# HKUST-Aerial-Robotics/ESVO

Hardware: AMD Instinct MI355X
Metric: mapped events/sec (stereo TS raster + block matching + LM depth refinement + fusion), events resident in HBM before the timed region; exactly K ticks between two synchronisations, i.e. including the fill and the drain of the two-deep tick pipeline (`sustained`: the same workload over 1600 ticks) (higher is better)
Workload: dtype f64

## Files before the change

esvo_amd/csrc/kernels_lm.hip:

```cpp
#define DEV_HOOKS_LM_TU
#include "common.hpp"
#include "dev_hooks.hpp"
#include "fdiv.hpp"
#include "lm_common.hpp"


namespace esvo {

#define LM_ROWS 7
#define LM_COLS 15

template <int CTRL>
__device__ inline double dpp_f64(double v) {
  const int lo = __double2loint(v), hi = __double2hiint(v);
  const int lo2 = __builtin_amdgcn_update_dpp(0, lo, CTRL, 0xf, 0xf, true);
  const int hi2 = __builtin_amdgcn_update_dpp(0, hi, CTRL, 0xf, 0xf, true);
  return __hiloint2double(hi2, lo2);
}
template <int CTRL>
__device__ inline int dpp_i32(int v) { return __builtin_amdgcn_update_dpp(0, v, CTRL, 0xf, 0xf, true); }
#define DPP_XOR1 0xB1
#define DPP_XOR2 0x4E
#define DPP_HALF_MIRROR 0x141
#define DPP_MIRROR 0x140
#define DPP_SHL1 0x101

__device__ inline double grp_sum(double v) {
  v = v + dpp_f64<DPP_XOR1>(v);
  v = v + dpp_f64<DPP_XOR2>(v);
  v = v + dpp_f64<DPP_HALF_MIRROR>(v);
  v = v + dpp_f64<DPP_MIRROR>(v);
  return v;
}
__device__ inline int grp_sum_int(int v) {
  v += dpp_i32<DPP_XOR1>(v);
  v += dpp_i32<DPP_XOR2>(v);
  v += dpp_i32<DPP_HALF_MIRROR>(v);
  v += dpp_i32<DPP_MIRROR>(v);
  return v;
}
__device__ inline double grp_min(double v) {
  v = fmin(v, dpp_f64<DPP_XOR1>(v));
  v = fmin(v, dpp_f64<DPP_XOR2>(v));
  v = fmin(v, dpp_f64<DPP_HALF_MIRROR>(v));
  v = fmin(v, dpp_f64<DPP_MIRROR>(v));
  return v;
}
template <bool WIDE>
struct Lay {
  static constexpr int RL = WIDE ? 2 : LM_ROWS;
};
__device__ inline double hop_f64(double v, int k) {
  const u32 lo = (u32)__double2loint(v), hi = (u32)__double2hiint(v);
  u32 l2, h2;
  if (k == 2) {
    l2 = __builtin_amdgcn_permlane32_swap(lo, lo, false, false)[0];
    h2 = __builtin_amdgcn_permlane32_swap(hi, hi, false, false)[0];
  } else if (k == 1) {
    l2 = __builtin_amdgcn_permlane16_swap(lo, lo, false, false)[0];
    h2 = __builtin_amdgcn_permlane16_swap(hi, hi, false, false)[0];
  } else {
    l2 = __builtin_amdgcn_permlane16_swap(lo, lo, false, false)[1];
    h2 = __builtin_amdgcn_permlane16_swap(hi, hi, false, false)[1];
  }
  return __hiloint2double((int)h2, (int)l2);
}
#define LM_WIDE_LAST_ROW_LANE 32
__device__ inline double bcast_f64(double v, int lane) {
  return __hiloint2double(__builtin_amdgcn_readlane(__double2hiint(v), lane), __builtin_amdgcn_readlane(__double2loint(v), lane));
}
template <bool WIDE>
__device__ inline double patch_sum(const double* t, int rg) {
  if constexpr (!WIDE) {
    double a = t[0];
#pragma unroll
    for (int y = 1; y < LM_ROWS; ++y) a = a + t[y];
    return grp_sum(a);
  } else {
    double a = t[0] + t[1];
    a = (hop_f64(a, 1) + t[0]) + t[1];
    a = (hop_f64(a, 2) + t[0]) + t[1];
    a = hop_f64(a, 3) + t[0];
    (void)rg;
    return bcast_f64(grp_sum(a), LM_WIDE_LAST_ROW_LANE);
  }
}
template <bool WIDE>
__device__ inline int match_sum_int(int v) {
  v = grp_sum_int(v);
  if constexpr (WIDE)
    v = (__builtin_amdgcn_readlane(v, 0) + __builtin_amdgcn_readlane(v, 16)) + (__builtin_amdgcn_readlane(v, 32) + __builtin_amdgcn_readlane(v, 48));
  return v;
}
template <bool WIDE>
__device__ inline double match_min(double v) {
  v = grp_min(v);
  if constexpr (WIDE) v = fmin(fmin(bcast_f64(v, 0), bcast_f64(v, 16)), fmin(bcast_f64(v, 32), bcast_f64(v, 48)));
  return v;
}
template <bool WIDE>
__device__ inline double patch_dot(const double* a, const double* b, int rg) {
  double t[Lay<WIDE>::RL];
#pragma unroll
  for (int y = 0; y < Lay<WIDE>::RL; ++y) t[y] = a[y] * b[y];
  return patch_sum<WIDE>(t, rg);
}

__device__ inline double in_vgpr(double x) {
  asm volatile("" : "+v"(x));
  return x;
}

struct LmProblem {
  double T[12];
  double cx, cy;
  double ray[3];
  __amdgpu_buffer_rsrc_t tsL;
  __amdgpu_buffer_rsrc_t tsR;
  const double* cam;
  int c;
  int rg;
  int vy0, vy1;
  DEV_LM_PROBLEM_FIELDS
};

struct PatchGeom { int ulx, uly; double q1, q2, q3, q4; bool ok; };
__device__ inline PatchGeom interp_geom(const DevParams& p, double lx, double ly) {
  PatchGeom g;
  const int hx = (LM_COLS - 1) / 2, hy = (LM_ROWS - 1) / 2;
  const double fx = floor(lx), fy = floor(ly);
  const int l1 = (int)fx, l0 = (int)fy;
  g.ulx = l1 - hx;
  g.uly = l0 - hy;
  const int drx = l1 + hx, dry = l0 + hy;
  g.ok = (int)(g.ulx >= 0) & (int)(g.uly >= 0) & (int)(drx < p.W) & (int)(dry < p.H) & (int)(g.uly + LM_ROWS < p.H) & (int)(g.ulx + LM_COLS < p.W);
  g.q1 = (fx + 1.0) - lx;
  g.q2 = lx - fx;
  g.q3 = (fy + 1.0) - ly;
  g.q4 = ly - fy;
  return g;
}
template <bool WIDE>
struct LmCache {
  float l[Lay<WIDE>::RL + 1], r[Lay<WIDE>::RL + 1];
  int vl, vr;
  __device__ inline void clear() {
#pragma unroll
    for (int y = 0; y <= Lay<WIDE>::RL; ++y) l[y] = r[y] = 0.f;
    vl = vr = 0x7fffffff;
  }
};
__device__ inline float dpp_shl1_f32(float v) { return __int_as_float(dpp_i32<DPP_SHL1>(__float_as_int(v))); }
template <bool WIDE>
__device__ inline void interp_column(__amdgpu_buffer_rsrc_t img, int W, const PatchGeom& g, int c, int rg, double* tau, float* cs,
                                     int& cvoff) {
  constexpr int RL = Lay<WIDE>::RL;
  const int voff = (g.uly + (WIDE ? 2 * rg : 0)) * W + g.ulx + c;
  if (__ballot(voff != cvoff) != 0ull) {
#pragma unroll
    for (int y = 0; y <= RL; ++y) cs[y] = (float)(int)__builtin_amdgcn_raw_buffer_load_b8(img, voff, y * W, 0);
    cvoff = voff;
  }
  double R[RL + 1];
#pragma unroll
  for (int y = 0; y <= RL; ++y) {
    const float s0 = cs[y];
    const float s1 = dpp_shl1_f32(s0);
    R[y] = g.q1 * (double)s0 + g.q2 * (double)s1;
  }
#pragma unroll
  for (int y = 0; y < RL; ++y) tau[y] = g.q3 * R[y] + g.q4 * R[y + 1];
}

template <bool WIDE, bool L2, bool COUNT = false, bool BAND = false>
__device__ bool lm_eval(const DevParams& p, const LmProblem& pr, LmCache<WIDE>& cc, double x, double* fv, int* n_iter = nullptr,
                        bool* viol = nullptr) {
  int iters = 0;
  constexpr int RL = Lay<WIDE>::RL;
  bool el[RL];
#pragma unroll
  for (int y = 0; y < RL; ++y) el[y] = pr.c < LM_COLS && (!WIDE || 2 * pr.rg + y < LM_ROWS);
  const double nu = in_vgpr(p.td_nu);
  DEV_LM_EVAL(pr);
  if constexpr (WIDE) asm volatile("" ::: "memory");
  double prv[3], pl[3];
  {
    const double z = 1.0 / x;
#pragma unroll
    for (int r = 0; r < 3; ++r) prv[r] = z * pr.ray[r] - pr.cam[24 + r];
  }
#pragma unroll
  for (int r = 0; r < 3; ++r)
    pl[r] = ((pr.T[r * 4 + 0] * prv[0] + pr.T[r * 4 + 1] * prv[1]) + pr.T[r * 4 + 2] * prv[2]) + pr.T[r * 4 + 3];
  double x1u, x1v, x2u, x2v;
  {
    double hL[3], hR[3];
#pragma unroll
    for (int r = 0; r < 3; ++r) {
      const double* PL = pr.cam + r * 4;
      const double* PR = pr.cam + 12 + r * 4;
      hL[r] = ((PL[0] * pl[0] + PL[1] * pl[1]) + PL[2] * pl[2]) + PL[3];
      hR[r] = ((PR[0] * pl[0] + PR[1] * pl[1]) + PR[2] * pl[2]) + PR[3];
    }
    if (__double_as_longlong(hL[2]) == __double_as_longlong(hR[2]) &&
        (unsigned)(((__double2hiint(hL[2]) >> 20) & 0x7ff) - 923) <= 200u) {
      Recip rz;
      rz.b = hL[2];
      rz.y = recip_refined(hL[2]);
      x1u = div_fast(hL[0], rz);
      x1v = div_fast(hL[1], rz);
      x2u = div_fast(hR[0], rz);
      x2v = div_fast(hR[1], rz);
    } else {
      x1u = hL[0] / hL[2];
      x1v = hL[1] / hL[2];
      x2u = hR[0] / hR[2];
      x2v = hR[1] / hR[2];
    }
  }
  const int hx = (LM_COLS - 1) / 2, hy = (LM_ROWS - 1) / 2;
  const double wlo = (double)hx, whi = (double)(p.W - hx), vlo = (double)hy, vhi = (double)(p.H - hy);
  const bool inside = (int)(x1u >= wlo) & (int)(x1u <= whi) & (int)(x1v >= vlo) & (int)(x1v <= vhi) &
                      (int)(x2u >= wlo) & (int)(x2u <= whi) & (int)(x2v >= vlo) & (int)(x2v <= vhi);
  const PatchGeom g1 = interp_geom(p, x1u, x1v), g2 = interp_geom(p, x2u, x2v);
  const bool okw = inside & g1.ok & g2.ok;
  if constexpr (BAND) {
    const bool bad = (int)okw & ((int)(g1.uly < pr.vy0) | (int)(g1.uly + LM_ROWS >= pr.vy1) | (int)(g2.uly < pr.vy0) | (int)(g2.uly + LM_ROWS >= pr.vy1));
    *viol = *viol | bad;
  }
  double tau1[RL], tau2[RL], r[RL], r2[RL];
  interp_column<WIDE>(pr.tsL, p.W, g1, pr.c, pr.rg, tau1, cc.l, cc.vl);
  interp_column<WIDE>(pr.tsR, p.W, g2, pr.c, pr.rg, tau2, cc.r, cc.vr);
  if (!okw) {
    double f = 255;
    if constexpr (!L2) {
      const double q = f / p.td_scale;
      const double weight = (nu + 1) / (nu + q * q);
      f = sqrt(weight) * f;
    }
#pragma unroll
    for (int y = 0; y < RL; ++y) fv[y] = el[y] ? f : 0.0;
    if constexpr (COUNT) *n_iter = 0;
    return false;
  }
  if constexpr (L2) {
#pragma unroll
    for (int y = 0; y < RL; ++y) fv[y] = el[y] ? (tau1[y] - tau2[y]) : 0.0;
    return false;
  }
  int knz = 0;
  double minabs = 1e300, r2max = 0;
  double r2n[RL];
#pragma unroll
  for (int y = 0; y < RL; ++y) {
    r[y] = el[y] ? (tau1[y] - tau2[y]) : 0.0;
    r2[y] = r[y] * r[y];
    r2n[y] = r2[y] * (nu + 1);
    r2max = fmax(r2max, r2[y]);
    if (r[y] != 0) { knz++; minabs = fmin(minabs, fabs(r[y])); }
  }
  const int knz_lane = knz;
  knz = match_sum_int<WIDE>(knz);
  DEV_LM_FIRST_EVAL_KNZ(pr, knz);
  minabs = match_min<WIDE>(minabs);
  const double scale2_0 = in_vgpr(p.td_scale2);
  double s2;
  const int e_r2max = (__double2hiint(r2max) >> 20) & 0x7ff;
  const bool r2_tight = knz_lane == 0 || (minabs * minabs >= 0x1p-100 && r2max < 0x1p98);
  const bool nu_mid = nu >= 0x1p-100 && nu < 0x1p100;
  bool lane_ok = r2_tight && nu_mid;
  if (!lane_ok) {
    bool r2_ok = true;
#pragma unroll
    for (int y = 0; y < RL; ++y) r2_ok = r2_ok && fdiv_ok(r2[y]);
    lane_ok = r2_ok && fdiv_ok(nu) && nu > 0 && fdiv_ok(r2max * (nu + 1));
  }
  const int N = LM_ROWS * LM_COLS;
  const bool tight = match_sum_int<WIDE>((r2_tight && nu_mid) ? 0 : 1) == 0;
  if ((double)knz * (nu + 1) / (double)N <= 0.94 && minabs >= 1e-6) {
    s2 = scale2_0;
    DEV_LM_SHORTCUT(pr);
  } else {
    double s1 = scale2_0;
    const Recip rN = make_recip((double)N);
    bool done = false;
    if (tight) {
      while ((unsigned)(((__double2hiint(s1) >> 20) & 0xfff) - 923) <= 200u) {
        if constexpr (COUNT) ++iters;
        DEV_LM_SCALE_ITER(pr);
        Recip rs1;
        rs1.b = s1;
        rs1.y = recip_refined(s1);
        double t[RL];
#pragma unroll
        for (int y = 0; y < RL; ++y) {
          Recip rd;
          rd.b = nu + div_fast(r2[y], rs1);
          rd.y = recip_refined(rd.b);
          t[y] = div_fast(r2n[y], rd);
        }
        const double sum = patch_sum<WIDE>(t, pr.rg);
        if (sum == 0) { s2 = scale2_0; done = true; break; }
        s2 = div_fast(sum, rN);
        const double rel = div_fast(fabs(s2 - s1), rs1);
        if (!(rel > 0.05)) { done = true; break; }
        s1 = s2;
      }
    }
    while (!done) {
      if constexpr (COUNT) ++iters;
      DEV_LM_SCALE_ITER(pr);
      double t[RL];
      const Recip rs1 = make_recip(s1);
      const int e_s1 = (__double2hiint(s1) >> 20) & 0x7ff;
      if (lane_ok && rs1.fast && s1 > 0 && e_r2max - e_s1 < 300) {
#pragma unroll
        for (int y = 0; y < RL; ++y)
          t[y] = div_fast(r2n[y], make_recip(nu + div_fast(r2[y], rs1)));
      } else {
#pragma unroll
        for (int y = 0; y < RL; ++y) t[y] = (r[y] != 0) ? r2[y] * (nu + 1) / (nu + r2[y] / s1) : 0.0;
      }
      const double sum = patch_sum<WIDE>(t, pr.rg);
      if (sum == 0) { s2 = scale2_0; break; }
      s2 = div_by(sum, rN);
      const double rel = div_by(fabs(s2 - s1), rs1);
      if (!(rel > 0.05)) break;
      s1 = s2;
    }
  }
  if (tight && (unsigned)(((__double2hiint(s2) >> 20) & 0xfff) - 923) <= 200u) {
    Recip rs2;
    rs2.b = s2;
    rs2.y = recip_refined(s2);
    const double nu1 = nu + 1;
#pragma unroll
    for (int y = 0; y < RL; ++y) {
      Recip rd;
      rd.b = nu + div_fast(r2[y], rs2);
      rd.y = recip_refined(rd.b);
      fv[y] = sqrt_moderate(div_fast(nu1, rd)) * r[y];
    }
    if constexpr (COUNT) *n_iter = iters;
    return true;
  }
  const Recip rs2 = make_recip(s2);
  const bool fast2 = lane_ok && rs2.fast && s2 > 0 && e_r2max - ((__double2hiint(s2) >> 20) & 0x7ff) < 300;
#pragma unroll
  for (int y = 0; y < RL; ++y) {
    fv[y] = fast2 ? sqrt_moderate(div_fast(nu + 1, make_recip(nu + div_fast(r2[y], rs2)))) * r[y]
                  : sqrt((nu + 1) / (nu + r2[y] / s2)) * r[y];
  }
  if constexpr (COUNT) *n_iter = iters;
  return false;
}

#ifndef LM_WAVES
#define LM_WAVES 2
#endif
#ifndef LM_BLOCK
#define LM_BLOCK 64
#endif
#ifndef LM_WIDE_WAVES
#define LM_WIDE_WAVES 3
#endif
#ifndef LM_WIDE_MAX
#define LM_WIDE_MAX 40000u
#endif
struct LmSplit {
  double* fvec0;
  double* fnorm0;
  u32* meta;
  u32* order;
  u32* hist;
};
#define LM_SPLIT_BINS 64
#define LM_SPLIT_STRIPES 32
__device__ inline u32 lm_split_stripe(u32 slot) { return (slot >> 2) & (LM_SPLIT_STRIPES - 1); }

template <bool WIDE, bool L2 = false, int STAGE = 0, bool PAIR = false, bool BAND = false>
__global__ void __launch_bounds__(PAIR ? 128 : LM_BLOCK, WIDE ? LM_WIDE_WAVES : LM_WAVES) lm_refine_kernel(LmArgs a, DevParams p, u32* n_solved, LmSplit sp) {
  static_assert(!PAIR || (WIDE && !L2 && STAGE == 0), "the pair layout is a variant of the wide one");
  static_assert(!BAND || (STAGE == 0 && !PAIR), "routed band launches are single launches of the narrow or the wide layout");
  constexpr int RL = Lay<WIDE>::RL;
  __shared__ double lds_pair[PAIR ? 2 : 1][2][RL][64];
  __shared__ int lds_pair_tight[PAIR ? 2 : 1][2];
  const int wv = PAIR ? (int)(threadIdx.x >> 6) : 0;
  const int ln = threadIdx.x & 63;
  __shared__ double lds_cam[28];
  if (threadIdx.x < 27) {
    const int i = threadIdx.x;
    lds_cam[i] = i < 12 ? p.camL.P[i] : (i < 24 ? p.camR.P[i - 12] : p.camL.Kinv_t[i - 24]);
  }
  __syncthreads();
  const u32 pos = WIDE ? blockIdx.x : (blockIdx.x * LM_BLOCK + threadIdx.x) >> 4;
  const int c = threadIdx.x & 15;
  const int drow = (threadIdx.x >> 4) & 3;
  const int rg = WIDE ? (drow ^ (drow >> 1)) : 0;
  const bool lead = WIDE ? threadIdx.x == 0 : c == 0;
  u32 M = *a.n_matches;
  if (M > a.max_matches) M = a.max_matches;
  bool active = pos < M;
  u32 s = pos;
  if constexpr (STAGE == 2) {
    if (blockIdx.x < 2 * LM_SPLIT_STRIPES * LM_SPLIT_BINS / LM_BLOCK) sp.hist[blockIdx.x * LM_BLOCK + threadIdx.x] = 0u;
    s = active ? sp.order[pos] : 0xffffffffu;
  }
  if (STAGE != 2 && !active && lead && s < a.max_matches) a.out_flags[s] = 0u;
  if (__ballot(active) == 0) return;
  const bool probe = STAGE != 1 && a.clk != nullptr && threadIdx.x == 0 && blockIdx.x % CLK_STRIDE == 0u;
  if (probe) {
    u64* sc = a.clk + CLK_SCRATCH + 2 * (size_t)(blockIdx.x / CLK_STRIDE);
    sc[0] = __builtin_readcyclecounter();
    sc[1] = __builtin_amdgcn_s_memrealtime();
  }
  u32 j = 0;
  esvo_match_t m;
  m.x_left[0] = m.x_left[1] = -1e9; m.inv_depth = 1.0; m.pose_idx = 0; m.cost = 0; m.disp = 0; m.event_idx = 0;
  if (active) {
    j = a.dense ? s : stride_item(s, M, (u32)p.num_threads);
    u32 jm = j;
    if constexpr (WIDE) { if (a.match_index) jm = a.match_index[j]; }
    m = a.matches[jm];
  }
  LmProblem pr;
  pr.cx = m.x_left[0];
  pr.cy = m.x_left[1];
  {
    const int n_bytes = p.W * p.H;
    pr.tsL = __builtin_amdgcn_make_buffer_rsrc(const_cast<uint8_t*>(a.tsL), 0, n_bytes, 0x00020000);
    pr.tsR = __builtin_amdgcn_make_buffer_rsrc(const_cast<uint8_t*>(a.tsR), 0, n_bytes, 0x00020000);
  }
#pragma unroll
  for (int r3 = 0; r3 < 3; ++r3)
    pr.ray[r3] = (p.camL.Kinv[r3 * 3 + 0] * pr.cx + p.camL.Kinv[r3 * 3 + 1] * pr.cy) + p.camL.Kinv[r3 * 3 + 2];
  pr.cam = lds_cam;
  pr.c = c;
  pr.rg = rg;
  pr.vy0 = a.vy0; pr.vy1 = a.vy1;
  bool viol = false;
  DEV_LM_SET_SLOT(pr, active ? s : 0xffffffffu);
  {
    double Tlw[16], Tlv[16];
    rigid_inverse(a.T_world_obs, Tlw);
    mat4_mul(Tlw, a.pose_T + (size_t)m.pose_idx * 16, Tlv);
#pragma unroll
    for (int i = 0; i < 12; ++i) pr.T[i] = Tlv[i];
  }
  const int N = LM_ROWS * LM_COLS;
  const double ftol = 1e-6, xtol = 1e-6, gtol = 0., factor = 100.;
  const double eps = 2.220446049250313e-16;
  const double sqrt_eps = 1.4901161193847656e-08;
  const int maxfev = p.lm_maxfev;

  double x = m.inv_depth;
  double fvec[RL], out[RL];
  LmCache<WIDE> cc;
  cc.clear();
  double fnorm = 0., par = 0., diag = 0., xnorm = 0., delta = 0., r = 0., qtf = 0., gnorm = 0.;
  double h = 0., xnew = 0., wa1 = 0., pnorm = 0.;
  int nfev = 1, iter = 1, iteration = 0, optState = 0;
  int phase = 0;
  bool need_step = false;
  bool fvec_tight = false;
  double xe = x;
  double xs = 0.;
  int xpar = 0;
  bool have_spec = false;
  if constexpr (STAGE == 1) {
    int n_it = 0;
    const bool tgt = lm_eval<WIDE, L2, true>(p, pr, cc, x, out, &n_it);
    const double f0 = sqrt(patch_dot<WIDE>(out, out, rg));
    if (active) {
      double* dst = sp.fvec0 + (size_t)s * (LM_ROWS * 16) + c;
#pragma unroll
      for (int y = 0; y < RL; ++y) dst[y * 16] = out[y];
      if (lead) {
        const u32 key = n_it < LM_SPLIT_BINS - 1 ? (u32)n_it : (u32)(LM_SPLIT_BINS - 1);
        sp.fnorm0[s] = f0;
        sp.meta[s] = key | (tgt ? 0x100u : 0u);
        atomicAdd(&sp.hist[lm_split_stripe(s) * LM_SPLIT_BINS + key], 1u);
      }
    }
    return;
  }
  if constexpr (STAGE == 2) {
    if (active) {
      const double* src = sp.fvec0 + (size_t)s * (LM_ROWS * 16) + c;
#pragma unroll
      for (int y = 0; y < RL; ++y) fvec[y] = src[y * 16];
      fnorm = sp.fnorm0[s];
      fvec_tight = (sp.meta[s] & 0x100u) != 0;
    } else {
#pragma unroll
      for (int y = 0; y < RL; ++y) fvec[y] = 0.0;
    }
    par = 0.;
    iter = 1;
    phase = 1;
    h = sqrt_eps * fabs(x);
    if (h == 0.) h = sqrt_eps;
    xe = x + h;
  }
  DEV_LM_JAC_DECL
  while (true) {
    if (need_step) {
      const double pstep = lm_lmpar2(r, diag, qtf, delta, par);
      wa1 = -pstep;
      xnew = x + wa1;
      pnorm = fabs(diag * wa1);
      if (iter == 1) delta = (pnorm < delta) ? pnorm : delta;
      xe = xnew;
      need_step = false;
    }
    bool out_tight;
    if constexpr (PAIR) {
      const bool reuse = phase == 1 && have_spec && __double_as_longlong(xe) == __double_as_longlong(xs);
      if (reuse) {
#pragma unroll
        for (int y = 0; y < RL; ++y) out[y] = lds_pair[xpar][1][y][ln];
        out_tight = lds_pair_tight[xpar][1] != 0;
        have_spec = false;
      } else {
        const bool side = phase != 1;
        if (side) {
          double hs = sqrt_eps * fabs(xe);
          if (hs == 0.) hs = sqrt_eps;
          xs = xe + hs;
        }
        const bool t_mine = lm_eval<WIDE, L2>(p, pr, cc, (side && wv) ? xs : xe, out);
        out_tight = t_mine;
        if (side) {
          xpar ^= 1;
#pragma unroll
          for (int y = 0; y < RL; ++y) lds_pair[xpar][wv][y][ln] = out[y];
          if (ln == 0) lds_pair_tight[xpar][wv] = t_mine ? 1 : 0;
          __syncthreads();
#pragma unroll
          for (int y = 0; y < RL; ++y) out[y] = lds_pair[xpar][0][y][ln];
          out_tight = lds_pair_tight[xpar][0] != 0;
          have_spec = true;
        }
      }
    } else {
      out_tight = lm_eval<WIDE, L2, false, BAND>(p, pr, cc, xe, out, nullptr, &viol);
    }
    int status = -1;
    bool outer_tail = false;
    if (phase == 0) {
      fvec_tight = out_tight;
#pragma unroll
      for (int y = 0; y < RL; ++y) fvec[y] = out[y];
      fnorm = sqrt(patch_dot<WIDE>(fvec, fvec, rg));
      par = 0.;
      iter = 1;
    } else if (phase == 1) {
      DEV_LM_JAC_PASS(pr, active, x);
      double fjac[RL];
      {
        const Recip rh = make_recip(h);
        if (out_tight && fvec_tight && rh.fast) {
#pragma unroll
          for (int y = 0; y < RL; ++y) fjac[y] = div_fast(out[y] - fvec[y], rh);
        } else {
#pragma unroll
          for (int y = 0; y < RL; ++y) fjac[y] = (out[y] - fvec[y]) / h;
        }
      }
      nfev += 2;
      const double wa2n = sqrt(patch_dot<WIDE>(fjac, fjac, rg));
      const double jtf = patch_dot<WIDE>(fjac, fvec, rg);
      r = wa2n;
      const double fvec0 = WIDE ? bcast_f64(fvec[0], 0) : __shfl(fvec[0], 0, 16);
      qtf = (r != 0.) ? jtf / r : fvec0;
      if (iter == 1) {
        diag = (wa2n == 0.) ? 1. : wa2n;
        xnorm = fabs(diag * x);
        delta = factor * xnorm;
        if (delta == 0.) delta = factor;
      }
      gnorm = 0.;
      if (fnorm != 0.)
        if (wa2n != 0.) { const double g = fabs(r * (qtf / fnorm) / wa2n); gnorm = (gnorm < g) ? g : gnorm; }
      if (gnorm <= gtol) {
        status = 4;
        outer_tail = true;
      } else {
        diag = (diag < wa2n) ? wa2n : diag;
        need_step = true;
        phase = 2;
      }
    } else {
      ++nfev;
      const double fnorm1 = sqrt(patch_dot<WIDE>(out, out, rg));
      double actred = -1.;
      if (0.1 * fnorm1 < fnorm) actred = 1. - (fnorm1 / fnorm) * (fnorm1 / fnorm);
      const double wa3 = r * wa1;
      const double t1 = fabs(wa3) / fnorm, temp1 = t1 * t1;
      const double t2 = sqrt(par) * pnorm / fnorm, temp2 = t2 * t2;
      const double prered = temp1 + temp2 / 0.5;
      const double dirder = -(temp1 + temp2);
      double ratio = 0.;
      if (prered != 0.) ratio = actred / prered;
      if (ratio <= 0.25) {
        double temp = 0.5;
        if (actred >= 0.) temp = 0.5;
        if (actred < 0.) temp = 0.5 * dirder / (dirder + 0.5 * actred);
        if (0.1 * fnorm1 >= fnorm || temp < 0.1) temp = 0.1;
        const double pn = pnorm / 0.1;
        delta = temp * ((pn < delta) ? pn : delta);
        par /= temp;
      } else if (!(par != 0. && ratio < 0.75)) {
        delta = pnorm / 0.5;
        par = 0.5 * par;
      }
      if (ratio >= 1e-4) {
        x = xnew;
        fvec_tight = out_tight;
#pragma unroll
        for (int y = 0; y < RL; ++y) fvec[y] = out[y];
        xnorm = fabs(diag * x);
        fnorm = fnorm1;
        ++iter;
      }
      if (fabs(actred) <= ftol && prered <= ftol && 0.5 * ratio <= 1. && delta <= xtol * xnorm) status = 3;
      else if (fabs(actred) <= ftol && prered <= ftol && 0.5 * ratio <= 1.) status = 1;
      else if (delta <= xtol * xnorm) status = 2;
      else if (nfev >= maxfev) status = 5;
      else if (fabs(actred) <= eps && prered <= eps && 0.5 * ratio <= 1.) status = 6;
      else if (delta <= eps * xnorm) status = 7;
      else if (gnorm <= eps) status = 8;
      if (status >= 0 || !(ratio < 1e-4)) outer_tail = true;
      else need_step = true;
    }
    if (phase == 0) {
      phase = 1;
    } else if (outer_tail) {
      iteration++;
      if (iteration >= p.lm_max_iter) break;
      if (status == 2 || status == 3) {
        if (optState == 0) optState++;
        else break;
      }
      phase = 1;
    }
    if (phase == 1) {
      h = sqrt_eps * fabs(x);
      if (h == 0.) h = sqrt_eps;
      xe = x + h;
    }
  }

  if (probe) {
    const u64* sc = a.clk + CLK_SCRATCH + 2 * (size_t)(blockIdx.x / CLK_STRIDE);
    const u64 c1 = __builtin_readcyclecounter(), r1 = __builtin_amdgcn_s_memrealtime();
    u32 xcc;
    asm volatile("s_getreg_b32 %0, hwreg(HW_REG_XCC_ID, 0, 4)" : "=s"(xcc));
    xcc &= CLK_XCDS - 1;
    atomicAdd(&a.clk[2 * xcc], c1 - sc[0]);
    atomicAdd(&a.clk[2 * xcc + 1], r1 - sc[1]);
    atomicAdd(&a.clk[CLK_SAMPLES], 1ull);
  }
  if (!active || !lead) return;
  if constexpr (BAND) { if (viol) atomicAdd(a.halo_viol, 1u); }
  const bool solved = !(x <= 0.001);
  bool keep = solved;
  if (solved) {
    atomicAdd(n_solved, 1u);
    const double invJtJ = (r != 0.) ? (1. / r) * (1. / r) : 0.;
    double variance;
    if constexpr (L2) {
      variance = fnorm * fnorm / (double)(N - 1) * invJtJ;
      if (variance < 1e-6) variance = 1e-6;
    } else {
      variance = p.td_stdvar2 * invJtJ;
    }
    const double residual = fnorm * fnorm;
    DevPoint o;
    o.row = (u32)(size_t)floor(pr.cy);
    o.col = (u32)(size_t)floor(pr.cx);
    o.x[0] = pr.cx;
    o.x[1] = pr.cy;
    cam2World(p.camL, pr.cx, pr.cy, x, o.p_cam);
    DEV_PERTURB_POINT(o, s);
    o.inv_depth = x;

    o.scale2 = L2 ? 0.0 : variance * (p.td_nu - 2) / p.td_nu;
    o.nu = L2 ? 0.0 : p.td_nu;
    o.variance = variance;
    o.residual = residual;
    o.age = 0;
    o.pose_idx = m.pose_idx;
    o.seq = j;
    if (a.cull)
      keep = variance <= p.var_thr && residual <= p.cost_thr && x > -1e-6 && x >= p.invdepth_min && x <= p.invdepth_max;
    if (keep) a.out_slots[s] = o;
  }
  a.out_flags[s] = keep ? 1u : 0u;
}

__global__ void __launch_bounds__(256) lm_order_kernel(const u32* __restrict__ n_matches, u32 max_matches, LmSplit sp) {
  __shared__ u32 base[LM_SPLIT_STRIPES][LM_SPLIT_BINS];
  __shared__ u32 tot[LM_SPLIT_BINS];
  if (threadIdx.x < LM_SPLIT_BINS) {
    const int k = threadIdx.x;
    u32 run = 0;
    for (int st = 0; st < LM_SPLIT_STRIPES; ++st) {
      base[st][k] = run;
      run += sp.hist[st * LM_SPLIT_BINS + k];
    }
    tot[k] = run;
  }
  __syncthreads();
  u32 off = 0;
  if (threadIdx.x < LM_SPLIT_BINS)
    for (int k = LM_SPLIT_BINS - 1; k > (int)threadIdx.x; --k) off += tot[k];
  __syncthreads();
  if (threadIdx.x < LM_SPLIT_BINS)
    for (int st = 0; st < LM_SPLIT_STRIPES; ++st) base[st][threadIdx.x] += off;
  __syncthreads();
  u32 M = *n_matches;
  if (M > max_matches) M = max_matches;
  const u32 s = blockIdx.x * blockDim.x + threadIdx.x;
  if (s >= M) return;
  const u32 key = sp.meta[s] & 0xffu, st = lm_split_stripe(s);
  u32* fill = sp.hist + LM_SPLIT_STRIPES * LM_SPLIT_BINS;
  sp.order[base[st][key] + atomicAdd(&fill[st * LM_SPLIT_BINS + key], 1u)] = s;
}

void launch_lm_refine_any(const LmArgs& a, const DevParams& p, u32* n_solved, hipStream_t s);
bool lm_launch_is_wide(u32 max_matches, const DevParams& p) {
  return max_matches > 0 && p.wx == LM_COLS && p.wy == LM_ROWS && p.ls_norm != ESVO_LSNORM_L2 && max_matches <= LM_WIDE_MAX && LM_BLOCK == 64;
}
void launch_lm_refine(const LmArgs& a, const DevParams& p, u32* n_solved, hipStream_t s) {
  if (a.max_matches == 0) return;
  if (p.wx != LM_COLS || p.wy != LM_ROWS) { launch_lm_refine_any(a, p, n_solved, s); return; }
  LmSplit sp;
  sp.fvec0 = a.split_fvec0; sp.fnorm0 = a.split_fnorm0; sp.meta = a.split_meta; sp.order = a.split_order; sp.hist = a.split_hist;
  const u32 groups_per_block = LM_BLOCK / 16;
  const u32 blocks = (a.max_matches + groups_per_block - 1) / groups_per_block;
  if (p.ls_norm == ESVO_LSNORM_L2) {
    if (a.halo_viol) hipLaunchKernelGGL((lm_refine_kernel<false, true, 0, false, true>), dim3(blocks), dim3(LM_BLOCK), 0, s, a, p, n_solved, sp);
    else hipLaunchKernelGGL((lm_refine_kernel<false, true, 0>), dim3(blocks), dim3(LM_BLOCK), 0, s, a, p, n_solved, sp);
    return;
  }
  if (a.halo_viol) {
    if (a.max_matches <= LM_WIDE_MAX && LM_BLOCK == 64)
      hipLaunchKernelGGL((lm_refine_kernel<true, false, 0, false, true>), dim3(a.max_matches), dim3(64), 0, s, a, p, n_solved, sp);
    else
      hipLaunchKernelGGL((lm_refine_kernel<false, false, 0, false, true>), dim3(blocks), dim3(LM_BLOCK), 0, s, a, p, n_solved, sp);
    return;
  }
  if (a.max_matches <= LM_WIDE_MAX && LM_BLOCK == 64) {
    if (a.pair)
      hipLaunchKernelGGL((lm_refine_kernel<true, false, 0, true>), dim3(a.max_matches), dim3(128), 0, s, a, p, n_solved, sp);
    else
      hipLaunchKernelGGL((lm_refine_kernel<true, false, 0>), dim3(a.max_matches), dim3(64), 0, s, a, p, n_solved, sp);
    return;
  }
  if (a.split_fvec0 && !a.dense) {
    hipLaunchKernelGGL((lm_refine_kernel<false, false, 1>), dim3(blocks), dim3(LM_BLOCK), 0, s, a, p, n_solved, sp);
    hipLaunchKernelGGL(lm_order_kernel, dim3((a.max_matches + 255) / 256), dim3(256), 0, s, a.n_matches, a.max_matches, sp);
    hipLaunchKernelGGL((lm_refine_kernel<false, false, 2>), dim3(blocks), dim3(LM_BLOCK), 0, s, a, p, n_solved, sp);
    return;
  }
  hipLaunchKernelGGL((lm_refine_kernel<false, false, 0>), dim3(blocks), dim3(LM_BLOCK), 0, s, a, p, n_solved, sp);
}

__global__ void __launch_bounds__(256) compact_points_kernel(const DevPoint* __restrict__ slots, const u32* __restrict__ flags,
                                                             const u32* __restrict__ prefix, const u32* __restrict__ n_in,
                                                             u32 max_n, DevPoint* __restrict__ out) {
  const u32 s = blockIdx.x * blockDim.x + threadIdx.x;
  u32 n = *n_in;
  if (n > max_n) n = max_n;
  if (s >= n || !flags[s]) return;
  DevPoint o = slots[s];
  o.seq = prefix[s];
  out[prefix[s]] = o;
}
void launch_compact_points(const DevPoint* slots, const u32* flags, const u32* prefix, const u32* n_in, u32 max_n,
                           DevPoint* out, hipStream_t s) {
  if (max_n == 0) return;
  hipLaunchKernelGGL(compact_points_kernel, dim3((max_n + 255) / 256), dim3(256), 0, s, slots, flags, prefix, n_in, max_n,
                     out);
}

}
```

Before: 156.3 million.

## Skip redundant Jacobian re-evaluation when x unchanged and simplify residual tightness checks

In the LM loop, when an outer iteration ends without accepting a step (x unchanged since the last Jacobian), the previous Jacobian is reused instead of re-running the finite-difference evaluations. A gnorm<=gtol case fast-forwards the remaining iterations directly. The first-eval tightness test drops the per-lane r2max reduction and the cross-lane vote, using the already-reduced knz/minabs and a fixed exponent. This saves residual evaluations and reductions, but relies on the skipped state being identical and changes which lanes take the tight path.

```diff
diff --git a/esvo_amd/csrc/kernels_lm.hip b/esvo_amd/csrc/kernels_lm.hip
--- a/esvo_amd/csrc/kernels_lm.hip
+++ b/esvo_amd/csrc/kernels_lm.hip
@@ -249,34 +249,33 @@
     return false;
   }
   int knz = 0;
-  double minabs = 1e300, r2max = 0;
+  double minabs = 1e300;
   double r2n[RL];
 #pragma unroll
   for (int y = 0; y < RL; ++y) {
     r[y] = el[y] ? (tau1[y] - tau2[y]) : 0.0;
     r2[y] = r[y] * r[y];
     r2n[y] = r2[y] * (nu + 1);
-    r2max = fmax(r2max, r2[y]);
     if (r[y] != 0) { knz++; minabs = fmin(minabs, fabs(r[y])); }
   }
-  const int knz_lane = knz;
   knz = match_sum_int<WIDE>(knz);
   DEV_LM_FIRST_EVAL_KNZ(pr, knz);
   minabs = match_min<WIDE>(minabs);
   const double scale2_0 = in_vgpr(p.td_scale2);
   double s2;
-  const int e_r2max = (__double2hiint(r2max) >> 20) & 0x7ff;
-  const bool r2_tight = knz_lane == 0 || (minabs * minabs >= 0x1p-100 && r2max < 0x1p98);
+  const int e_r2max = 1023 + 17;
+  const bool r2_tight = knz == 0 || minabs * minabs >= 0x1p-100;
   const bool nu_mid = nu >= 0x1p-100 && nu < 0x1p100;
-  bool lane_ok = r2_tight && nu_mid;
+  const bool tight = r2_tight && nu_mid;
+  bool lane_ok = tight;
   if (!lane_ok) {
     bool r2_ok = true;
-#pragma unroll
-    for (int y = 0; y < RL; ++y) r2_ok = r2_ok && fdiv_ok(r2[y]);
+    double r2max = 0;
+#pragma unroll
+    for (int y = 0; y < RL; ++y) { r2_ok = r2_ok && fdiv_ok(r2[y]); r2max = fmax(r2max, r2[y]); }
     lane_ok = r2_ok && fdiv_ok(nu) && nu > 0 && fdiv_ok(r2max * (nu + 1));
   }
   const int N = LM_ROWS * LM_COLS;
-  const bool tight = match_sum_int<WIDE>((r2_tight && nu_mid) ? 0 : 1) == 0;
   if ((double)knz * (nu + 1) / (double)N <= 0.94 && minabs >= 1e-6) {
     s2 = scale2_0;
     DEV_LM_SHORTCUT(pr);
@@ -463,6 +462,7 @@
   int phase = 0;
   bool need_step = false;
   bool fvec_tight = false;
+  int jac_iter = 0;
   double xe = x;
   double xs = 0.;
   int xpar = 0;
@@ -534,7 +534,7 @@
           xpar ^= 1;
 #pragma unroll
           for (int y = 0; y < RL; ++y) lds_pair[xpar][wv][y][ln] = out[y];
-          if (ln == 0) lds_pair_tight[xpar][wv] = t_mine ? 1 : 0;
+          lds_pair_tight[xpar][wv] = t_mine ? 1 : 0;
           __syncthreads();
 #pragma unroll
           for (int y = 0; y < RL; ++y) out[y] = lds_pair[xpar][0][y][ln];
@@ -582,6 +582,7 @@
       gnorm = 0.;
       if (fnorm != 0.)
         if (wa2n != 0.) { const double g = fabs(r * (qtf / fnorm) / wa2n); gnorm = (gnorm < g) ? g : gnorm; }
+      jac_iter = iter;
       if (gnorm <= gtol) {
         status = 4;
         outer_tail = true;
@@ -637,12 +638,32 @@
       phase = 1;
     } else if (outer_tail) {
       iteration++;
-      if (iteration >= p.lm_max_iter) break;
-      if (status == 2 || status == 3) {
+      bool done = iteration >= p.lm_max_iter;
+      if (!done && (status == 2 || status == 3)) {
         if (optState == 0) optState++;
-        else break;
-      }
+        else done = true;
+      }
+      const bool again = !done && jac_iter == iter;
+      if (again && gnorm <= gtol) {
+        do {
+          DEV_LM_JAC_PASS(pr, active, x);
+          nfev += 2;
+          iteration++;
+        } while (iteration < p.lm_max_iter);
+        done = true;
+      }
+      if (done) break;
       phase = 1;
+      if (again) {
+        DEV_LM_JAC_PASS(pr, active, x);
+        nfev += 2;
+        if (iter == 1) {
+          delta = factor * xnorm;
+          if (delta == 0.) delta = factor;
+        }
+        need_step = true;
+        phase = 2;
+      }
     }
     if (phase == 1) {
       h = sqrt_eps * fabs(x);
```

Result: no change. 155.8 million (-0.3%).
